# wathiede/pbrt

Measured on AMD Instinct MI355X. Metric: Msamples/sec (rays/sec) at 1/2/4/8 GPUs; PSNR vs CPU reference, higher is better.
Workload: dtype f32

## Files before the change

### include/pbrt_hip_debug.h

```cpp
#ifndef PBRT_HIP_DEBUG_H
#define PBRT_HIP_DEBUG_H
#include "pbrt_hip.h"
#ifdef __cplusplus
extern "C" {
#endif

int pbrt_hip_scene_canonical_info(const pbrt_hip_scene *scene, uint32_t *ready, double *build_ms);
int pbrt_hip_scene_optimize_cost(const pbrt_hip_scene *scene, double *before, double *after, uint32_t *undone);
int pbrt_hip_scene_export_quads(const pbrt_hip_scene *scene, uint32_t *quads, uint32_t cap_nodes, uint32_t *n_quads,
                                uint32_t *order);
int pbrt_hip_scene_export_bvh(const pbrt_hip_scene *scene, uint32_t *nodes , uint32_t *order);
int pbrt_hip_scene_walk_info(const pbrt_hip_scene *scene, uint32_t *quad_nodes, uint32_t *stack_need);
int pbrt_hip_render_stack_plan(uint32_t stack_need, uint32_t *lds_rows, uint32_t *waves_per_cu, uint32_t *overflow_entries);
int pbrt_hip_rccl_library(char *path, size_t cap);
int pbrt_hip_bvh_build_host(const float *P, uint32_t n_verts, const uint32_t *idx, uint32_t n_tris,
                            uint32_t *nodes , uint32_t *order, uint32_t *n_nodes,
                            uint32_t *depth);

int pbrt_hip_quad_build_host(const float *P, uint32_t n_verts, const uint32_t *idx, uint32_t n_tris, int split_leaves,
                             uint32_t *quads, uint32_t cap_nodes, uint32_t *n_quads, uint32_t *stack_need);
#define PBRT_HIP_TREE_SAH 0u
#define PBRT_HIP_TREE_REINSERT 2u
#define PBRT_HIP_TREE_DEFAULT 0xffffffffu
int pbrt_hip_quad_build_host_ex(const float *P, uint32_t n_verts, const uint32_t *idx, uint32_t n_tris, int split_leaves,
                                uint32_t tree, uint32_t *quads, uint32_t cap_nodes, uint32_t *n_quads, uint32_t *stack_need,
                                uint32_t *order, float *root_box, uint32_t *n_refs, float *exact_boxes);

void pbrt_hip_sobol_matrices(uint32_t *out_4096_words);
int pbrt_hip_envmap_tables(const float *rgb, uint32_t width, uint32_t height, float *marginal, float *conditional, float *p_uv);
int pbrt_hip_envmap_eval_host(const float *rgb, uint32_t width, uint32_t height, const float world_to_light[9], int64_t n, const float *u12,
                              float *d, uint32_t *texel, float *le, float *pdf);
int pbrt_hip_envmap_eval_device(pbrt_hip_scene *scene, int64_t n, const float *u12, float *d, uint32_t *texel, float *le, float *pdf);

#define PBRT_HIP_BLOCK_SIN 0u
#define PBRT_HIP_BLOCK_COS 1u
#define PBRT_HIP_BLOCK_ATAN_POS 2u
// ... 25 lines not shown
```

### pbrt_amd/_lib.py

```python
import ctypes as C
import os

from .build import LIB_PATH


class Material(C.Structure):
    _fields_ = [("type", C.c_uint32), ("k", C.c_float * 3), ("le", C.c_float * 3), ("kd_tex", C.c_uint32)]


class Texture(C.Structure):
    _fields_ = [("type", C.c_uint32), ("tex1", C.c_float * 3), ("tex2", C.c_float * 3), ("su", C.c_float), ("sv", C.c_float),
                ("du", C.c_float), ("dv", C.c_float), ("pad", C.c_uint32 * 5)]


class EnvMap(C.Structure):
    _fields_ = [("type", C.c_uint32), ("width", C.c_uint32), ("height", C.c_uint32), ("reserved", C.c_uint32), ("rgb", C.POINTER(C.c_float)),
                ("world_to_light", C.c_float * 9), ("pad", C.c_uint32)]


class Normals(C.Structure):
    _fields_ = [("type", C.c_uint32), ("n_tris", C.c_uint32), ("reserved", C.c_uint32 * 2), ("tri_n", C.POINTER(C.c_float)),
                ("pad", C.c_uint32 * 10)]


# ... 31 lines not shown
        ("nodes_visited", C.c_uint64), ("tris_tested", C.c_uint64), ("kernel_ms", C.c_double),
        ("samples", C.c_uint64),
    ]


_f, _u32, _i32, _i64, _u64, _vp = C.c_float, C.c_uint32, C.c_int32, C.c_int64, C.c_uint64, C.c_void_p
_pf, _pu32, _pi32, _pi64, _pu64, _pu8 = (C.POINTER(t) for t in (_f, _u32, _i32, _i64, _u64, C.c_uint8))
SYMBOLS = {
    "pbrt_hip_device_count": (C.c_int, []),
    "pbrt_hip_last_error": (C.c_char_p, []),
    "pbrt_hip_version": (C.c_char_p, []),
    "pbrt_hip_build_id": (C.c_char_p, []),
    "pbrt_hip_scene_create": (C.c_int, [C.POINTER(SceneDesc), C.c_int, C.POINTER(_vp)]),
    "pbrt_hip_scene_create_ex": (C.c_int, [C.POINTER(SceneDesc), C.c_int, _u32, C.POINTER(_vp)]),
    "pbrt_hip_scene_build_info": (C.c_int, [_vp, _pu32, C.POINTER(C.c_double)]),
    "pbrt_hip_scene_canonical_info": (C.c_int, [_vp, _pu32, C.POINTER(C.c_double)]),
    "pbrt_hip_scene_optimize_info": (C.c_int, [_vp, _pu32, _pu32, C.POINTER(C.c_double)]),
    "pbrt_hip_rccl_library": (C.c_int, [C.c_char_p, C.c_size_t]),
    "pbrt_hip_scene_optimize_cost": (C.c_int, [_vp, C.POINTER(C.c_double), C.POINTER(C.c_double), _pu32]),
    "pbrt_hip_scene_export_quads": (C.c_int, [_vp, _pu32, _u32, _pu32, _pu32]),
    "pbrt_hip_scene_destroy": (None, [_vp]),
    "pbrt_hip_scene_info": (C.c_int, [_vp, _pu32, _pu32, _pu32, _pu64]),
    "pbrt_hip_render_stack_plan": (C.c_int, [C.c_uint32, _pu32, _pu32, _pu32]),
    "pbrt_hip_scene_export_bvh": (C.c_int, [_vp, _pu32, _pu32]),
    "pbrt_hip_scene_walk_info": (C.c_int, [_vp, _pu32, _pu32]),
    "pbrt_hip_bvh_build_host": (C.c_int, [_pf, _u32, _pu32, _u32, _pu32, _pu32, _pu32, _pu32]),
    "pbrt_hip_quad_build_host": (C.c_int, [_pf, _u32, _pu32, _u32, C.c_int, _pu32, _u32, _pu32, _pu32]),
    "pbrt_hip_quad_build_host_ex": (C.c_int, [_pf, _u32, _pu32, _u32, C.c_int, _u32, _pu32, _u32, _pu32, _pu32, _pu32, _pf, _pu32, _pf]),
    "pbrt_hip_render": (C.c_int, [_vp, C.POINTER(RenderDesc), _pf, C.POINTER(Stats)]),
    "pbrt_hip_render_device": (C.c_int, [_vp, C.POINTER(RenderDesc), _vp, _vp]),
    "pbrt_hip_render_prepare": (C.c_int, [_vp, C.POINTER(RenderDesc)]),
    "pbrt_hip_render_wait": (C.c_int, [_vp, C.POINTER(Stats)]),
    "pbrt_hip_film_assemble_device": (C.c_int, [_vp, _vp, _u32, _u32, _vp, _vp]),
    "pbrt_hip_render_buffer_bytes": (_i64, [_vp, C.POINTER(RenderDesc)]),
    "pbrt_hip_render_acc": (C.c_int, [_vp, C.POINTER(RenderDesc), _pi64, C.POINTER(Stats)]),
    "pbrt_hip_film_from_acc_device": (C.c_int, [_vp, _vp, _vp, _vp]),
    "pbrt_hip_film_from_acc": (None, [_pi64, _i64, _pf]),
    "pbrt_hip_sobol_matrices": (None, [_pu32]),
    "pbrt_hip_slab_floats": (_i64, [_i32, _i32, _pf, _u32, _u32]),
    "pbrt_hip_slab_pixel_index": (C.c_int, [_i32, _i32, _pf, _u32, _u32, _pi64]),
    "pbrt_hip_multi_create": (C.c_int, [C.POINTER(SceneDesc), C.c_int, _u32, C.POINTER(_vp)]),
    "pbrt_hip_multi_gpus": (C.c_int, [_vp]),
    "pbrt_hip_multi_render": (C.c_int, [_vp, C.POINTER(RenderDesc), _pf, C.POINTER(Stats)]),
    "pbrt_hip_multi_film_device": (C.c_int, [_vp, C.POINTER(_vp)]),
    "pbrt_hip_multi_destroy": (None, [_vp]),
    "pbrt_hip_render_multi": (C.c_int, [C.POINTER(SceneDesc), C.POINTER(RenderDesc), C.c_int, _pf, C.POINTER(Stats)]),
# ... 71 lines not shown
```

### pbrt_amd/csrc/capi_render.cpp

```cpp
#include <hip/hip_runtime.h>

#include <cmath>
#include <cstdio>
#include <cstdlib>
#include <cstring>
#include <algorithm>
#include <limits>
#include <string>
#include <vector>

#include "../../include/pbrt_hip.h"
#include "capi_internal.hpp"
#include "device_types.h"
#include "host_math.hpp"
#include "rgb_xyz.hpp"

using namespace pbrt_hip;

namespace pbrt_hip {
namespace {
inline float filter_radius(float w) { return w == 0.f ? 0.5f : w; }
inline bool filter_is_wide(float rx, float ry) { return rx != 0.5f || ry != 0.5f; }
void sample_bounds(const int32_t c[4], float rx, float ry, int32_t sb[4]) {
  sb[0] = (int32_t)std::floor(((float)c[0] + 0.5f) - rx);
// ... 46 lines not shown
  int32_t b[4];
  film_cropped_bounds(xres, yres, crop, b);
  return make_shard_bounds(b, rank, world);
}
struct TileRect {
  int32_t x0, y0, w, h;
};
TileRect super_tile(const Shard &sh, uint32_t rank, uint32_t world, uint32_t j) {
  const uint32_t t = rank + j * world;
  const int32_t x0 = (int32_t)(t % sh.stx) * 64, y0 = (int32_t)(t / sh.stx) * 64;
  return {x0, y0, sh.w - x0 < 64 ? sh.w - x0 : 64, sh.h - y0 < 64 ? sh.h - y0 : 64};
}

uint32_t tuning(const char *name, uint32_t dflt, long cap = 64) {
  const char *v = debug_knob(name);
  if (!v || !*v) return dflt;
  long x = std::strtol(v, nullptr, 10);
  return x < 0 ? 0u : (x > cap ? (uint32_t)cap : (uint32_t)x);
}
constexpr uint32_t kMinWalkers = 36, kMinWalkersShallow = 20, kShallowStackNeed = 16, kMinParked = 16;
constexpr uint32_t kRenderWavesPerCuSpheres = 12;
constexpr uint32_t kRenderWavesPerCuEnv = 16;
constexpr uint32_t kRenderWavesPerCuN = 16;
RenderStackPlan stack_plan(uint32_t quad_stack_need) {
  static const bool force_overflow = debug_knob("PBRT_HIP_FORCE_OVERFLOW_VARIANT") != nullptr;
  static const bool prefer_lds = debug_knob("PBRT_HIP_PREFER_LDS_STACK") != nullptr;
  return render_stack_plan(quad_stack_need, force_overflow, prefer_lds);
}
bool is_table_sampler(uint32_t sampler) { return sampler == PBRT_HIP_SAMPLER_SOBOL_ND || sampler == PBRT_HIP_SAMPLER_HALTON; }

int check_render_desc(const pbrt_hip_scene *s, const pbrt_hip_render_desc *r) {
  if (!s || !r) return fail(PBRT_HIP_ERR_INVALID, "render: null argument");
  if (r->spp_x == 0 || r->spp_y == 0) return fail(PBRT_HIP_ERR_INVALID, "render: spp_x and spp_y must be >= 1");
  if (r->world_size == 0 || r->rank >= r->world_size) return fail(PBRT_HIP_ERR_INVALID, "render: rank must be < world_size");
  if (r->integrator > PBRT_HIP_INTEGRATOR_PATH_MIS) return fail(PBRT_HIP_ERR_INVALID, "render: unknown integrator");
  if (r->sampler > PBRT_HIP_SAMPLER_HALTON) return fail(PBRT_HIP_ERR_INVALID, "render: unknown sampler");
  const bool counting = (r->flags & (PBRT_HIP_FLAG_COUNTERS | PBRT_HIP_FLAG_WALK_COUNTERS)) != 0u;
  if (is_table_sampler(r->sampler) && counting)
    return fail(PBRT_HIP_ERR_INVALID, "render: the counter flags are not available with the Sobol' / Halton samplers (samplers 2, 3)");
  if ((uint64_t)r->spp_x * (uint64_t)r->spp_y > PBRT_HIP_MAX_SPP)
    return fail(PBRT_HIP_ERR_LIMIT, "render: more than 2^20 samples per pixel");
  if (r->max_depth > PBRT_HIP_MAX_DEPTH) return fail(PBRT_HIP_ERR_LIMIT, "render: maxdepth above 1023");
  const float fx = filter_radius(r->filter_xwidth), fy = filter_radius(r->filter_ywidth);
  if (!(fx > 0.f) || !(fy > 0.f) || !std::isfinite(fx) || !std::isfinite(fy)) return fail(PBRT_HIP_ERR_INVALID, "render: the filter radii must be positive");
  if (fx > 16.f || fy > 16.f) return fail(PBRT_HIP_ERR_LIMIT, "render: filter radius above 16 pixels");
  const bool wide = filter_is_wide(fx, fy);
  if (wide && counting)
    return fail(PBRT_HIP_ERR_INVALID, "render: the counter flags need the default box filter (radius 0.5)");
  if (s->normals && counting)
    return fail(PBRT_HIP_ERR_LIMIT, "render: the counter flags are not available for a scene with shading normals");
// ... 16 lines not shown
  return PBRT_HIP_OK;
}

uint32_t partials_passes(uint32_t n_local, uint32_t n_chunks) {
  if (n_local == 0) return 1;
  const uint64_t cap_bytes = (uint64_t)std::max<uint32_t>(1u, tuning("PBRT_HIP_PARTIALS_CAP_KB", 2u << 20, 1l << 30)) << 10;
  const uint64_t per_tile = 4096ull * n_chunks * 16ull;
  uint64_t tiles = std::max<uint64_t>(1, cap_bytes / per_tile);
  tiles = std::min<uint64_t>(tiles, ((1ull << 32) - 1) / (4096ull * n_chunks));
  return (uint32_t)((n_local + tiles - 1) / tiles);
}
int render_launch(pbrt_hip_scene *s, const pbrt_hip_render_desc *r, const FilmGeom &fg, const Shard &sh, RenderLaunch *out) {
  RenderLaunch L{};
  L.spheres = s->dev.n_spheres > 0;
  L.counters = (r->flags & PBRT_HIP_FLAG_COUNTERS) ? kCountExact : ((r->flags & PBRT_HIP_FLAG_WALK_COUNTERS) ? kCountWalk : kCountNone);
  L.wide = fg.wide;
  L.table_sampler = is_table_sampler(r->sampler);
  L.mis = r->integrator == PBRT_HIP_INTEGRATOR_PATH_MIS;
  L.textured = s->textured;
  L.glass = s->glass;
  L.env = s->env;
  L.normals = s->normals;
  const bool shallow = s->dev.quad_stack_need <= kShallowStackNeed;
  L.plan = stack_plan(s->dev.quad_stack_need);
  L.lds_bytes = L.plan.rows * 256u;
  const bool default_path = L.counters == kCountNone && !L.wide && !L.table_sampler && !L.mis && !L.textured && !L.glass && !L.env && !L.normals;
  L.steps = default_path && !L.plan.overflow && shallow ? 2u : PBRT_STEPS_PER_CHECK;
  if (L.counters == kCountExact) {
    const int ce = ensure_canonical(s);
    if (ce) return ce;
    const uint32_t held = s->bvh.depth > 0 ? s->bvh.depth - 1 : 0;
    L.exact_rows = held > 40 ? 64 : held > 32 ? 40 : held > 26 ? 32 : held > 20 ? 26 : 20;
    L.lds_bytes = L.exact_rows * 512u;
  }
  L.waves_per_cu = (L.spheres || L.glass) ? std::min(kRenderWavesPerCuSpheres, L.plan.waves_per_cu) : L.plan.waves_per_cu;
  if (L.env) L.waves_per_cu = std::min(kRenderWavesPerCuEnv, L.plan.waves_per_cu);
  if (L.normals) L.waves_per_cu = std::min(kRenderWavesPerCuN, L.plan.waves_per_cu);
  L.chunk_shift = sample_chunk_shift(r->spp_x * r->spp_y);
  const uint32_t n_chunks = 1u << L.chunk_shift;
  L.passes = fg.wide ? 1u : partials_passes(sh.n_local, n_chunks);
  L.pass_tiles = (sh.n_local + L.passes - 1) / L.passes;
  if ((uint64_t)L.pass_tiles * 4096u * n_chunks >= (1ull << 32)) return fail(PBRT_HIP_ERR_LIMIT, "render: film too large for 32-bit item numbers");
  if ((uint64_t)r->world_size * L.passes >= (1ull << 32)) return fail(PBRT_HIP_ERR_LIMIT, "render: world_size x passes does not fit 32 bits");
  L.n_workgroups = std::min<uint32_t>(L.pass_tiles * 64u * n_chunks, std::max<uint32_t>(1u, tuning("PBRT_HIP_RENDER_WORKGROUPS", s->n_cu * L.waves_per_cu, 1 << 20)));
  L.min_walkers = tuning("PBRT_HIP_MIN_WALKERS", shallow ? kMinWalkersShallow : kMinWalkers);
  L.min_parked = tuning("PBRT_HIP_MIN_PARKED", kMinParked);
  *out = L;
  return PBRT_HIP_OK;
}
// ... 18 lines not shown
    if (s->d_partials.n / 4 > need) s->d_partials.release();
    HIP_TRY(s->d_partials.grow(need));
  }
  HIP_TRY(s->d_stack_overflow.grow((size_t)L.n_workgroups * 64 * L.plan.extra_entries));
  return PBRT_HIP_OK;
}
void scene_render_params(const pbrt_hip_scene *s, RenderParams *R) {
  R->tri_uv = s->d_tri_uv.p;
  R->textures = s->d_textures.p;
  R->glass = s->d_glass.p;
  R->env_texels = s->d_env_texels.p;
  R->env_marginal = s->d_env_marginal.p;
  R->env_conditional = s->d_env_conditional.p;
  R->env_w = s->env_w; R->env_h = s->env_h;
  for (int k = 0; k < 9; k++) R->env_m[k] = s->env_m[k];
  for (int k = 0; k < 3; k++) R->env_c[k] = s->env_c[k];
  R->tri_n = s->d_tri_n.p;
}
}

extern "C" {

int pbrt_hip_render_stack_plan(uint32_t stack_need, uint32_t *lds_rows, uint32_t *waves_per_cu, uint32_t *overflow_entries) {
  const RenderStackPlan p = stack_plan(stack_need);
  if (lds_rows) *lds_rows = p.rows;
  if (waves_per_cu) *waves_per_cu = p.waves_per_cu;
  if (overflow_entries) *overflow_entries = p.extra_entries;
  return PBRT_HIP_OK;
}

int pbrt_hip_envmap_eval_device(pbrt_hip_scene *s, int64_t n, const float *u12, float *d, uint32_t *texel, float *le, float *pdf) {
  if (!s) return fail(PBRT_HIP_ERR_INVALID, "envmap_eval_device: null scene");
  if (!s->env) return fail(PBRT_HIP_ERR_INVALID, "envmap_eval_device: the scene has no environment map");
  if (n < 0 || (n && !d)) return fail(PBRT_HIP_ERR_INVALID, "envmap_eval_device: null argument");
  if (n == 0) return PBRT_HIP_OK;
  return guarded([&]() -> int {
    HIP_TRY(hipSetDevice(s->device));
    DevBuf<float> d_u, d_d, d_le, d_pdf;
    DevBuf<uint32_t> d_texel;
    HIP_TRY(d_d.alloc(3 * (size_t)n));
    HIP_TRY(d_le.alloc(3 * (size_t)n));
    HIP_TRY(d_pdf.alloc((size_t)n));
    HIP_TRY(d_texel.alloc((size_t)n));
    if (u12) {
      HIP_TRY(d_u.alloc(2 * (size_t)n));
      HIP_TRY(hipMemcpyAsync(d_u.p, u12, 8 * (size_t)n, hipMemcpyHostToDevice, s->stream));
    } else {
      HIP_TRY(hipMemcpyAsync(d_d.p, d, 12 * (size_t)n, hipMemcpyHostToDevice, s->stream));
// ... 386 lines not shown
```

### pbrt_amd/csrc/device_types.h

```cpp
#pragma once
#include <stdint.h>

#include <hip/hip_runtime.h>

#include <cstdlib>

namespace pbrt_hip {

inline const char *debug_knob(const char *name) {
  const char *on = std::getenv("PBRT_HIP_DEBUG_KNOBS");
  if (!on || !*on || (on[0] == '0' && !on[1])) return nullptr;
  return std::getenv(name);
}

#ifdef PBRT_QUAD_LDS_STACK
constexpr uint32_t kQuadLdsStack = PBRT_QUAD_LDS_STACK, kQuadLdsStackOvf = PBRT_QUAD_LDS_STACK;
#else
constexpr uint32_t kQuadLdsStack = 40, kQuadLdsStackOvf = 30;
#endif
constexpr uint32_t kLdsGranule = 1280u;
constexpr uint32_t kLdsBytesPerCu = 160u * 1024u;
#ifndef PBRT_TRI_STRIDE
#define PBRT_TRI_STRIDE 4
#endif
constexpr uint32_t kTriStride = PBRT_TRI_STRIDE;
#ifndef PBRT_STEPS_PER_CHECK
#define PBRT_STEPS_PER_CHECK 3
#endif
#ifndef PBRT_RENDER_MAX_WAVES_PER_CU
#define PBRT_RENDER_MAX_WAVES_PER_CU 20
#endif
constexpr uint32_t kRenderMaxWavesPerCu = PBRT_RENDER_MAX_WAVES_PER_CU;

constexpr uint32_t kEmptyLeafRef = 0x80000000u;
constexpr uint32_t kLeafRef = 0x80000000u;

constexpr uint32_t kMaxSampleChunks = 16u, kMinSamplesPerChunk = 32u;
inline uint32_t sample_chunk_shift(uint32_t spp) {
  uint32_t kb = 0;
  while ((2u << kb) <= kMaxSampleChunks && (2u << kb) * kMinSamplesPerChunk <= spp) kb++;
  return kb;
}

constexpr uint32_t kSobolNdRequests = 64u;

struct RenderStackPlan {
  uint32_t rows;
  bool overflow;
  uint32_t waves_per_cu;
  uint32_t extra_entries;
};
inline RenderStackPlan render_stack_plan(uint32_t quad_stack_need, bool force_overflow, bool prefer_lds = false) {
  RenderStackPlan p;
  const uint32_t need_rows = quad_stack_need + 2u;
  auto waves = [](uint32_t rows) {
    const uint32_t bytes = (rows * 256u + kLdsGranule - 1u) / kLdsGranule * kLdsGranule, w = kLdsBytesPerCu / bytes;
    return w > kRenderMaxWavesPerCu ? kRenderMaxWavesPerCu : w;
  };
  p.rows = need_rows < 8u ? 8u : need_rows;
  p.overflow = force_overflow || need_rows > kQuadLdsStack || (waves(p.rows) < waves(kQuadLdsStackOvf) && !prefer_lds);
  if (p.overflow) p.rows = kQuadLdsStackOvf;
  p.waves_per_cu = waves(p.rows);
  p.extra_entries = p.overflow && need_rows > p.rows ? need_rows - p.rows : 0u;
  return p;
}
constexpr uint32_t kIntersectLdsStack = 20;
constexpr uint32_t kIntersectWavesPerWorkgroup = 4, kIntersectMaxWorkgroups = 256 * 16;
inline uint32_t intersect_workgroups(int64_t n_rays) {
  const int64_t w = (n_rays + 255) / 256;
  return w > kIntersectMaxWorkgroups ? kIntersectMaxWorkgroups : (uint32_t)w;
}
inline uint32_t intersect_overflow_entries(uint32_t quad_stack_need) {
  return quad_stack_need + 2u > kIntersectLdsStack ? quad_stack_need + 2u - kIntersectLdsStack : 0u;
}

struct DevScene {
  const uint4 *nodes;
  const uint4 *quads;
  uint32_t quad_stack_need;
  const float4 *tris;
  const float4 *mats;
  const float4 *lights;
  const float4 *spheres;
  uint32_t n_nodes, n_tris, n_spheres, n_lights;
  float n_lights_f;
// ... 124 lines not shown
```

### pbrt_amd/csrc/kernel_path.hpp

```cpp
#pragma once
#include "envmap_core.hpp"
#include "kernel_walk.hpp"

namespace pbrt_hip {
namespace {

__device__ __forceinline__ bool sample_light(const DevScene &S, uint32_t li, V3 po, V3 nf, V3 kd, float u1, float u2,
                                             float nLf, V3 &Ld, V3 &wi, float &tmax, const bool mis = false) {
  const float4 l0 = S.lights[5 * li];
  const float4 l3 = S.lights[5 * li + 3];
  const uint32_t type = __float_as_uint(l0.x);
  const V3 p0 = {l0.y, l0.z, l0.w};
  const V3 lc = xyz(l3);
  const V3 f = kd * kInvPi;
  if (type == 0u) {
    V3 dv = p0 - po;
    float dist2 = dot(dv, dv);
    if (!(dist2 > 0.f)) return false;
    float dist = sqrtf(dist2);
    wi = dv / dist;
    float cs = dot(wi, nf);
    if (!(cs > 0.f)) return false;
    float scale = (cs / dist2) * nLf;
    Ld = (f * lc) * scale;
// ... 75 lines not shown
    scale = scale * mis_weight_light(pl, pbl);
  }
  Ld = (f * (mk(R.env_c[0], R.env_c[1], R.env_c[2]) * xyz(tx))) * scale;
  tmax = kInf;
  return true;
}

enum : uint32_t { ST_NEW = 0, ST_CLOSEST = 1, ST_SHADOW = 2, ST_DONE = 3, ST_FETCH = 4 };

#ifndef PBRT_RENDER_WAVES_PER_SIMD
#define PBRT_RENDER_WAVES_PER_SIMD 5
#endif

struct PathState {
  V3 L, beta;
  V3 wi_next;
  Pcg rng;
  uint32_t s, bounces;
  bool specular, cont;
};
struct LaneRecords {
  char *base;
  uint32_t off;
};
constexpr int32_t kRecL = -2048, kRecBeta = -1024, kRecWi = 0, kRecLpend = 1024, kRecSum = 2048;
__device__ __forceinline__ float4 rec_load(const LaneRecords &r, int32_t k) {
  uint32_t o = r.off;
  asm volatile("" : "+v"(o));
  return *reinterpret_cast<const float4 *>(r.base + o + k);
}
__device__ __forceinline__ void rec_store(const LaneRecords &r, int32_t k, float4 v) {
  uint32_t o = r.off;
  asm volatile("" : "+v"(o));
  *reinterpret_cast<float4 *>(r.base + o + k) = v;
}
__device__ __forceinline__ void path_store(const LaneRecords &rec, const PathState &P) {
  rec_store(rec, kRecL, make_float4(P.L.x, P.L.y, P.L.z,
                                    __uint_as_float(P.s | (P.bounces << 20) | (P.specular ? 1u << 30 : 0u) | (P.cont ? 1u << 31 : 0u))));
  rec_store(rec, kRecBeta, make_float4(P.beta.x, P.beta.y, P.beta.z, __uint_as_float((uint32_t)P.rng.state)));
  rec_store(rec, kRecWi, make_float4(P.wi_next.x, P.wi_next.y, P.wi_next.z, __uint_as_float((uint32_t)(P.rng.state >> 32))));
}
__device__ __forceinline__ void path_load(const LaneRecords &rec, PathState &P) {
  const float4 a = rec_load(rec, kRecL), b = rec_load(rec, kRecBeta), c = rec_load(rec, kRecWi);
  P.L = {a.x, a.y, a.z};
  P.beta = {b.x, b.y, b.z};
  P.wi_next = {c.x, c.y, c.z};
  const uint32_t w = __float_as_uint(a.w);
  P.s = w & 0xfffffu;
  P.bounces = (w >> 20) & 0x3ffu;
  P.specular = (w >> 30) & 1u;
  P.cont = (w >> 31) & 1u;
  P.rng.state = (uint64_t)__float_as_uint(b.w) | ((uint64_t)__float_as_uint(c.w) << 32);
}

__device__ __forceinline__ uint32_t chunk_begin(uint32_t c, uint32_t spp, uint32_t kb) { return (c * spp) >> kb; }
__device__ __forceinline__ uint32_t mix32(uint32_t v) {
  v ^= v >> 16; v *= 0x7feb352du; v ^= v >> 15; v *= 0x846ca68bu; v ^= v >> 16;
  return v;
}
__device__ __forceinline__ float halton_dim(const uint32_t *tab, uint32_t d, uint32_t i, uint32_t key, uint32_t spp_mask) {
  const uint4 t = reinterpret_cast<const uint4 *>(tab)[d];
  const uint32_t b = t.x;
  uint32_t h = mix32(key + (d + 1u) * 0x9e3779b9u);
  if (b == 2u) return fminf(kOneMinusEps, (float)(__builtin_bitreverse32(i) ^ h) * 2.3283064365386963e-10f);
  uint32_t v = 0u, n = i, pw = 1u;
  do {
// ... 90 lines not shown
```

### pbrt_amd/csrc/kernels.hip

```cpp
#include "kernel_path.hpp"
#include "rgb_xyz.hpp"
#include "with_bools.hpp"

namespace pbrt_hip {
namespace {

template <bool SPH, bool COUNT, bool EXACT, int STACK, int STEPS = PBRT_STEPS_PER_CHECK, bool WIDE = false, bool SND = false>
__global__ void __launch_bounds__(64, (COUNT ? 1 : (SPH ? 3 : PBRT_RENDER_WAVES_PER_SIMD))) render_kernel(const DevScene S, const RenderParams R) {
  constexpr bool MIS = false, TEX = false, GLS = false;
  constexpr bool ENV = false;
  constexpr bool NRM = false;
  (void)MIS;
  (void)GLS;
  (void)ENV;
#include "render_body.inc"
}

#ifndef PBRT_INTERSECT_WAVES_PER_SIMD
#define PBRT_INTERSECT_WAVES_PER_SIMD 8
#endif
template <bool SPH, bool COUNT, int STACK>
__global__ void __launch_bounds__(256, (COUNT ? 1 : (SPH ? 4 : PBRT_INTERSECT_WAVES_PER_SIMD))) intersect_kernel(const DevScene S, const RayBatch B, const int any_hit) {
  __shared__ uint32_t lds_stack[4][COUNT ? STACK : kIntersectLdsStack][64];
  __shared__ float lds_tn[COUNT ? 4 : 1][COUNT ? STACK : 1][64];
  const uint32_t lane = threadIdx.x & 63u, wave = threadIdx.x >> 6;
  uint32_t *stk = &lds_stack[wave][0][lane];
  float *stkt = &lds_tn[COUNT ? wave : 0][0][lane];
  uint32_t *ovf = B.stack_overflow + ((size_t)blockIdx.x * 4u + (uint32_t)__builtin_amdgcn_readfirstlane(wave)) * B.stack_overflow_entries * 64u;
  const TravTuning tune = {B.min_walkers, B.min_parked};
  unsigned long long cn = 0, ct = 0;
  EXP_PROBE_INIT_BLOCK();
  const int64_t stride = (int64_t)gridDim.x * 256;
  int64_t next = (int64_t)blockIdx.x * 256 + threadIdx.x, idx = 0;
  bool have = false;
// ... 155 lines not shown
  };
  if (L.counters == kCountExact)
    return with_bools([&](auto SPH) {
      switch (L.exact_rows) {
        case 20: return go(render_kernel<SPH, true, true, 20>);
        case 26: return go(render_kernel<SPH, true, true, 26>);
        case 32: return go(render_kernel<SPH, true, true, 32>);
        case 40: return go(render_kernel<SPH, true, true, 40>);
        case 64: return go(render_kernel<SPH, true, true, 64>);
      }
      return hipErrorInvalidValue;
    }, L.spheres);
  if (L.glass || L.mis || L.textured || (L.table_sampler && L.wide)) return launch_render_x(S, R, L, st);
  const bool experiment = kExperimentLaunch && L.counters == kCountNone && !L.wide && !L.table_sampler;
  hipError_t e = hipSuccess;
  if (experiment && experiment_launch_begin(&e)) return e;
  e = with_bools([&](auto SPH, auto OVF, auto COUNT, auto SND, auto WIDE) {
    constexpr int STACK = OVF ? (int)kQuadLdsStackOvf : 0;
    if constexpr ((COUNT && (SND || WIDE)) || (SND && WIDE)) {
      return hipErrorInvalidValue;
    } else if constexpr (!COUNT && !SND && !WIDE && STACK == 0) {
      return go(L.steps == 2 ? render_kernel<SPH, false, false, 0, 2> : render_kernel<SPH, false, false, 0>);
    } else {
      return go(render_kernel<SPH, COUNT, false, STACK, PBRT_STEPS_PER_CHECK, WIDE, SND>);
    }
  }, L.spheres, L.plan.overflow, L.counters == kCountWalk, L.table_sampler, L.wide);
  if (experiment) experiment_launch_end(st);
  return e;
}

hipError_t launch_intersect(const DevScene &S, const RayBatch &B, bool any_hit, uint32_t bvh_depth, hipStream_t st) {
  if (B.n == 0) return hipSuccess;
  const dim3 grid(intersect_workgroups(B.n)), block(64 * kIntersectWavesPerWorkgroup);
  const hipError_t e = with_bools([&](auto SPH, auto COUNT) {
    hipLaunchKernelGGL((bvh_depth <= 32 ? intersect_kernel<SPH, COUNT, 32> : intersect_kernel<SPH, COUNT, 64>), grid, block, 0, st, S, B, any_hit ? 1 : 0);
    return hipGetLastError();
  }, S.n_spheres > 0, B.counters != nullptr);
  if (kExperimentLaunch) experiment_launch_end(st);
  return e;
}

hipError_t launch_pack_tris(const float *P, const uint32_t *idx, const uint16_t *mat_id, const uint32_t *order,
                            uint32_t n_prims, uint32_t n_tris, const float4 *spheres, float4 *tris, hipStream_t stream) {
  if (n_prims == 0) return hipSuccess;
  hipLaunchKernelGGL(pack_tris_kernel, dim3((n_prims + 255) / 256), dim3(256), 0, stream, P, idx, mat_id, order, n_prims, n_tris, spheres,
                     tris);
// ... 29 lines not shown
```

### pbrt_amd/csrc/kernels_env.hip

```cpp
#include "kernel_path.hpp"
#include "with_bools.hpp"

namespace pbrt_hip {
namespace {

#ifndef PBRT_ENV_WAVES_PER_SIMD
#define PBRT_ENV_WAVES_PER_SIMD 4
#endif
template <bool SPH, int STACK, bool MIS, bool TEX, bool SND>
__global__ void __launch_bounds__(64, PBRT_ENV_WAVES_PER_SIMD) render_kernel_env(const DevScene S, const RenderParams R) {
  constexpr bool COUNT = false, EXACT = false, WIDE = false, GLS = true, ENV = true;
  constexpr bool NRM = false;
  constexpr int STEPS = PBRT_STEPS_PER_CHECK;
#include "render_body.inc"
}

__global__ void envmap_eval_kernel(const RenderParams R, int64_t n, const float *u12, float *d, uint32_t *texel, float *le, float *pdf) {
  const int64_t i = (int64_t)blockIdx.x * blockDim.x + threadIdx.x;
  if (i >= n) return;
  const envmap::Map m = env_map(R);
  float st;
  uint32_t t;
  if (u12) {
    float x, y, z;
    t = envmap::sample(m, u12[2 * i], u12[2 * i + 1], &x, &y, &z, &st);
    d[3 * i] = x; d[3 * i + 1] = y; d[3 * i + 2] = z;
  } else {
    t = envmap::lookup(m, d[3 * i], d[3 * i + 1], d[3 * i + 2], &st);
  }
  const float4 tx = m.texels[t];
  if (texel) texel[i] = t;
  if (le) { le[3 * i] = tx.x; le[3 * i + 1] = tx.y; le[3 * i + 2] = tx.z; }
  if (pdf) pdf[i] = envmap::pdf_omega(tx.w, st);
}

// ... 20 lines not shown
```

### pbrt_amd/csrc/kernels_n.hip

```cpp
#include "kernel_path.hpp"
#include "with_bools.hpp"

namespace pbrt_hip {
namespace {

#ifndef PBRT_NRM_WAVES_PER_SIMD
#define PBRT_NRM_WAVES_PER_SIMD 4
#endif
template <bool SPH, int STACK, bool MIS, bool TEX, bool SND, bool ENV>
__global__ void __launch_bounds__(64, PBRT_NRM_WAVES_PER_SIMD) render_kernel_n(const DevScene S, const RenderParams R) {
  constexpr bool COUNT = false, EXACT = false, WIDE = false, GLS = true, NRM = true;
  constexpr int STEPS = PBRT_STEPS_PER_CHECK;
#include "render_body.inc"
}

__global__ void pack_nrm_kernel(const float *tri_n, const uint32_t *order, uint32_t n_prims, uint32_t n_tris, float4 *out) {
  const uint32_t slot = blockIdx.x * blockDim.x + threadIdx.x;
  if (slot >= n_prims) return;
  const uint32_t t = order[slot];
  for (int v = 0; v < 3; v++) {
    const float *q = tri_n + 9 * (size_t)t + 3 * v;
    out[3u * slot + v] = t < n_tris ? make_float4(q[0], q[1], q[2], 0.f) : make_float4(0.f, 0.f, 0.f, 0.f);
  }
}

__global__ void __launch_bounds__(256) shading_normal_eval_kernel(int64_t n, const float *in, float *out) {
  const int64_t i = (int64_t)blockIdx.x * blockDim.x + threadIdx.x;
  if (i >= n) return;
  const float *x = in + 17 * i;
  const V3 sn_n0 = mk(x[0], x[1], x[2]), sn_n1 = mk(x[3], x[4], x[5]), sn_n2 = mk(x[6], x[7], x[8]);
  const V3 ng = mk(x[9], x[10], x[11]);
  const float sn_b1 = x[12], sn_b2 = x[13];
  const V3 wo = mk(x[14], x[15], x[16]);
#include "shading_normal.inc"
// ... 30 lines not shown
```

### pbrt_amd/csrc/kernels_x.hip

```cpp
#include "kernel_path.hpp"
#include "with_bools.hpp"

namespace pbrt_hip {
namespace {

template <bool SPH, int STACK, bool MIS, bool TEX, bool SND, bool WIDE, bool GLS = false>
__global__ void __launch_bounds__(64, ((SPH || GLS) ? 3 : PBRT_RENDER_WAVES_PER_SIMD)) render_kernel_x(const DevScene S, const RenderParams R) {
  constexpr bool COUNT = false, EXACT = false;
  constexpr bool ENV = false;
  constexpr bool NRM = false;
  constexpr int STEPS = PBRT_STEPS_PER_CHECK;
  (void)ENV;
#include "render_body.inc"
}

}

hipError_t launch_render_x(const DevScene &S, const RenderParams &R, const RenderLaunch &L, hipStream_t st) {
  if (R.n_items == 0) return hipSuccess;
  if (L.counters != kCountNone) return hipErrorInvalidValue;
  return with_bools([&](auto SPH, auto OVF, auto MIS, auto TEX, auto SND, auto WIDE, auto GLS) {
    constexpr int STACK = OVF ? (int)kQuadLdsStackOvf : 0;
    if constexpr (GLS || MIS || TEX || (SND && WIDE)) {
      hipLaunchKernelGGL((render_kernel_x<SPH, STACK, MIS, TEX, SND, WIDE, GLS>), dim3(L.n_workgroups), dim3(64), L.lds_bytes, st, S, R);
      return hipGetLastError();
    } else {
      return hipErrorInvalidValue;
    }
  }, L.spheres, L.plan.overflow, L.mis, L.textured, L.table_sampler, L.wide, L.glass);
}

}
```

### pbrt_amd/csrc/render_body.inc

```
  extern __shared__ uint32_t lds_stack[];
  const uint32_t lane = threadIdx.x;
  uint32_t *stk = lds_stack + lane;
  float *stkt = reinterpret_cast<float *>(lds_stack + (EXACT ? STACK : 0) * 64) + lane;
  uint32_t *ovf = R.stack_overflow + (size_t)blockIdx.x * R.stack_overflow_entries * 64u;

  const int32_t W = R.sw, H = R.sh;
  const uint32_t stx = (uint32_t)(W + 63) >> 6;
  const uint64_t seq0 = R.seed * (uint64_t)R.seq_w * (uint64_t)R.seq_h;
  uint32_t item = 0;
  auto pixel_xy = [&](uint32_t q, int32_t &xr, int32_t &yr) {
    const uint32_t tsup = R.rank + (q >> 12) * R.world;
    const uint32_t ty = stx == 1u ? tsup : __umulhi(tsup, R.stx_recip), tx = tsup - ty * stx;
    xr = (int32_t)(tx * 64u + ((q >> 6) & 7u) * 8u + (q & 7u));
    yr = (int32_t)(ty * 64u + ((q >> 9) & 7u) * 8u + ((q >> 3) & 7u));
  };
  const uint32_t kb = R.chunk_shift, chunk_mask = (1u << kb) - 1u;
  auto item_pixel = [&](uint32_t it) { return ((it >> (6u + kb)) << 6) | (it & 63u); };
  auto slab_pos = [](uint32_t q) {
    return (size_t)(q >> 12) * 4096u + (((q >> 9) & 7u) * 8u + ((q >> 3) & 7u)) * 64u + ((q >> 6) & 7u) * 8u + (q & 7u);
  };
  const bool sobol = SND ? true : R.sampler == 1u;
  const bool halton = SND && R.sampler == 3u;
  const uint32_t spp = R.spp_x * R.spp_y;
  const uint32_t spp_mask = R.spp_mask;
  const uint32_t nL = S.n_lights;
  const float nLf = S.n_lights_f;
  const bool direct_only = R.integrator == 1u;
  const TravTuning tune = {R.min_walkers, R.min_parked};

  const LaneRecords rec = {reinterpret_cast<char *>(R.lane_state + (size_t)blockIdx.x * 320u + 128u), lane * 16u};
  uint32_t state = ST_FETCH;
  if (WIDE) wide_slots_clear(R.wide_slots, lane);
  uint32_t region = blockIdx.x % R.n_regions;
  unsigned long long c_cam = 0, c_bounce = 0, c_shadow = 0, c_nodes = 0, c_tris = 0;
  Trav T;
  T.o = mk(0.f, 0.f, 0.f);
  T.d = mk(0.f, 0.f, 1.f);
  T.tmax = 0.f;
  T.cur = kDone;
  T.sp = 0;
  T.any = 0;
  T.h = HitRec{kInf, kNoPrim, kNoPrim, 0.f, 0.f};

  EXP_PROBE_INIT(lane);
  for (;;) {
    EXP_PROBE_LANES(4, state != ST_DONE && T.cur == kDone);
    const bool serve = state != ST_DONE && T.cur == kDone;
    PathState P;
    bool launch = false, launch_any = false;
    V3 ro = T.o, rd = T.d;
    float rtmax = kInf;
    int32_t xr = 0, yr = 0;
    if (serve && state != ST_FETCH) {
      path_load(rec, P);
      pixel_xy(item_pixel(item), xr, yr);
      P.rng.inc = ((((seq0 + (uint64_t)(R.seq_y0 + yr) * (uint64_t)R.seq_w + (uint64_t)(R.seq_x0 + xr)) << kb) + ((item >> 6) & chunk_mask)) << 1) | 1u;
      PROBE_SEC(1);
      if (state != ST_NEW) {
        bool advance = false;
        if (state == ST_SHADOW) {
          EXP_DEBUG_PIXEL("HIP s %u   shadow Lpend %08x occluded %u tmax %a\n", P.s, __float_as_uint(rec_load(rec, kRecLpend).x), T.any >> 1, T.tmax);
          if (T.any != 3u) {
            const float4 lp = rec_load(rec, kRecLpend);
            P.L = P.L + mk(lp.x, lp.y, lp.z);
          }
          advance = true;
        } else {
          const HitRec h = T.h;
          const bool hit = h.prim != kNoPrim;
          EXP_DEBUG_PIXEL("HIP s %u bounce %u prim %u t %08x b1 %a b2 %a L %08x beta %08x\n", P.s, P.bounces, h.prim, __float_as_uint(h.t), h.b1, h.b2,
                          __float_as_uint(P.L.x), __float_as_uint(P.beta.x));
          EXP_DEBUG_PIXEL("HIP s %u   ray o %a %a %a d %a %a %a\n", P.s, T.o.x, T.o.y, T.o.z, T.d.x, T.d.y, T.d.z);
          V3 p = {0.f, 0.f, 0.f}, ng = {0.f, 0.f, 1.f};
          float4 m0 = {0.f, 0.f, 0.f, 0.f}, m1 = {0.f, 0.f, 0.f, 0.f};
          float tri_area = 0.f;
          float4 gl = {0.f, 0.f, 0.f, 1.f};
          const V3 wo = -T.d;
// ... 318 lines not shown
            const uint32_t sx = P.s - sy * R.spp_x;
            jx = fminf(((float)sx + u1) * R.inv_nx, kOneMinusEps);
            jy = fminf(((float)sy + u2) * R.inv_ny, kOneMinusEps);
          }
          const float fx = (float)(R.sx0 + xr) + jx, fy = (float)(R.sy0 + yr) + jy;
          if (WIDE) rec_store(rec, kRecSum, make_float4(fx, fy, 0.f, 0.f));
          const V3 dc = unit(mk(fx * S.cam_ax + S.cam_bx, fy * S.cam_ay + S.cam_by, 1.0f));
          rd = {(S.c2w[0] * dc.x + S.c2w[1] * dc.y) + S.c2w[2] * dc.z,
                (S.c2w[4] * dc.x + S.c2w[5] * dc.y) + S.c2w[6] * dc.z,
                (S.c2w[8] * dc.x + S.c2w[9] * dc.y) + S.c2w[10] * dc.z};
          ro = {S.c2w[3], S.c2w[7], S.c2w[11]};
          rtmax = kInf;
          P.L = {0.f, 0.f, 0.f};
          P.beta = {1.f, 1.f, 1.f};
          P.specular = false;
          P.bounces = 0;
          state = ST_CLOSEST;
          launch = true;
          launch_any = false;
          if (COUNT) c_cam++;
        }
      }
      PROBE_SEC(7);
      path_store(rec, P);
      EXP_RAY_LOG(launch, ro, rd, rtmax, launch_any);
      if (launch) trav_begin<EXACT>(S, T, stk, ro, rd, rtmax, launch_any, c_nodes);
    }
    PROBE_SEC(8);
    if (__ballot(state != ST_DONE) == 0ull) break;
    wave_prio(PBRT_PRIO_ARITH);
    trav_run<EXACT, COUNT, ((!EXACT && STACK != 0) ? (uint32_t)STACK : 0u), STEPS, SPH>(S, T, stk, stkt, ovf, state != ST_DONE, tune, c_nodes, c_tris);
    wave_prio(PBRT_PRIO_SERVICE);
    PROBE_SEC(0);
  }

  EXP_PROBE_FINI(lane);
  if (COUNT) {
    unsigned long long v[5] = {c_cam, c_bounce, c_shadow, c_nodes, c_tris};
    for (int i = 0; i < 5; i++) {
      unsigned long long x = v[i];
      for (int off = 32; off > 0; off >>= 1) x += __shfl_down(x, off, 64);
      if (lane == 0) atomicAdd(&R.counters[i], x);
    }
  }
```

Measured before the change: 454.8.

## Keep per-lane path records in LDS behind the traversal stack for overflow kernels

In the overflow-stack render kernel on the default path, the three per-lane path-state records (L, beta, wi) now live in LDS, placed after a shortened traversal stack, instead of in global lane_state memory. The goal is to replace global-memory loads and stores at each path service step with LDS accesses. In exchange, the LDS walk stack shrinks by 12 rows, so more stack entries spill to the global overflow area. The LDS budget per wave and the waves-per-CU calculation now include the record rows, and a host check verifies that the plan matches the kernel variant.

```diff
diff --git a/include/pbrt_hip_debug.h b/include/pbrt_hip_debug.h
--- a/include/pbrt_hip_debug.h
+++ b/include/pbrt_hip_debug.h
@@ -12,6 +12,8 @@
 int pbrt_hip_scene_export_bvh(const pbrt_hip_scene *scene, uint32_t *nodes , uint32_t *order);
 int pbrt_hip_scene_walk_info(const pbrt_hip_scene *scene, uint32_t *quad_nodes, uint32_t *stack_need);
 int pbrt_hip_render_stack_plan(uint32_t stack_need, uint32_t *lds_rows, uint32_t *waves_per_cu, uint32_t *overflow_entries);
+int pbrt_hip_render_stack_layout(uint32_t stack_need, uint32_t *stack_rows, uint32_t *record_bytes, uint32_t *waves_per_cu,
+                                 uint32_t *overflow_entries);
 int pbrt_hip_rccl_library(char *path, size_t cap);
 int pbrt_hip_bvh_build_host(const float *P, uint32_t n_verts, const uint32_t *idx, uint32_t n_tris,
                             uint32_t *nodes , uint32_t *order, uint32_t *n_nodes,
diff --git a/pbrt_amd/_lib.py b/pbrt_amd/_lib.py
--- a/pbrt_amd/_lib.py
+++ b/pbrt_amd/_lib.py
@@ -77,6 +77,7 @@
     "pbrt_hip_scene_destroy": (None, [_vp]),
     "pbrt_hip_scene_info": (C.c_int, [_vp, _pu32, _pu32, _pu32, _pu64]),
     "pbrt_hip_render_stack_plan": (C.c_int, [C.c_uint32, _pu32, _pu32, _pu32]),
+    "pbrt_hip_render_stack_layout": (C.c_int, [C.c_uint32, _pu32, _pu32, _pu32, _pu32]),
     "pbrt_hip_scene_export_bvh": (C.c_int, [_vp, _pu32, _pu32]),
     "pbrt_hip_scene_walk_info": (C.c_int, [_vp, _pu32, _pu32]),
     "pbrt_hip_bvh_build_host": (C.c_int, [_pf, _u32, _pu32, _u32, _pu32, _pu32, _pu32, _pu32]),
diff --git a/pbrt_amd/csrc/capi_render.cpp b/pbrt_amd/csrc/capi_render.cpp
--- a/pbrt_amd/csrc/capi_render.cpp
+++ b/pbrt_amd/csrc/capi_render.cpp
@@ -92,10 +92,10 @@
 constexpr uint32_t kRenderWavesPerCuSpheres = 12;
 constexpr uint32_t kRenderWavesPerCuEnv = 16;
 constexpr uint32_t kRenderWavesPerCuN = 16;
-RenderStackPlan stack_plan(uint32_t quad_stack_need) {
+RenderStackPlan stack_plan(uint32_t quad_stack_need, bool lds_records) {
   static const bool force_overflow = debug_knob("PBRT_HIP_FORCE_OVERFLOW_VARIANT") != nullptr;
   static const bool prefer_lds = debug_knob("PBRT_HIP_PREFER_LDS_STACK") != nullptr;
-  return render_stack_plan(quad_stack_need, force_overflow, prefer_lds);
+  return render_stack_plan(quad_stack_need, force_overflow, prefer_lds, lds_records);
 }
 bool is_table_sampler(uint32_t sampler) { return sampler == PBRT_HIP_SAMPLER_SOBOL_ND || sampler == PBRT_HIP_SAMPLER_HALTON; }
 
@@ -158,9 +158,9 @@
   L.env = s->env;
   L.normals = s->normals;
   const bool shallow = s->dev.quad_stack_need <= kShallowStackNeed;
-  L.plan = stack_plan(s->dev.quad_stack_need);
-  L.lds_bytes = L.plan.rows * 256u;
   const bool default_path = L.counters == kCountNone && !L.wide && !L.table_sampler && !L.mis && !L.textured && !L.glass && !L.env && !L.normals;
+  L.plan = stack_plan(s->dev.quad_stack_need, default_path);
+  L.lds_bytes = (L.plan.rows + L.plan.record_rows) * 256u;
   L.steps = default_path && !L.plan.overflow && shallow ? 2u : PBRT_STEPS_PER_CHECK;
   if (L.counters == kCountExact) {
     const int ce = ensure_canonical(s);
@@ -225,8 +225,17 @@
 extern "C" {
 
 int pbrt_hip_render_stack_plan(uint32_t stack_need, uint32_t *lds_rows, uint32_t *waves_per_cu, uint32_t *overflow_entries) {
-  const RenderStackPlan p = stack_plan(stack_need);
+  const RenderStackPlan p = stack_plan(stack_need, false);
   if (lds_rows) *lds_rows = p.rows;
+  if (waves_per_cu) *waves_per_cu = p.waves_per_cu;
+  if (overflow_entries) *overflow_entries = p.extra_entries;
+  return PBRT_HIP_OK;
+}
+
+int pbrt_hip_render_stack_layout(uint32_t stack_need, uint32_t *stack_rows, uint32_t *record_bytes, uint32_t *waves_per_cu, uint32_t *overflow_entries) {
+  const RenderStackPlan p = stack_plan(stack_need, true);
+  if (stack_rows) *stack_rows = p.rows;
+  if (record_bytes) *record_bytes = p.record_rows * 256u;
   if (waves_per_cu) *waves_per_cu = p.waves_per_cu;
   if (overflow_entries) *overflow_entries = p.extra_entries;
   return PBRT_HIP_OK;
diff --git a/pbrt_amd/csrc/device_types.h b/pbrt_amd/csrc/device_types.h
--- a/pbrt_amd/csrc/device_types.h
+++ b/pbrt_amd/csrc/device_types.h
@@ -18,6 +18,15 @@
 #else
 constexpr uint32_t kQuadLdsStack = 40, kQuadLdsStackOvf = 30;
 #endif
+constexpr uint32_t kPathRecordRows = 12u;
+#ifdef PBRT_PATH_RECORDS_HBM
+constexpr bool kLdsPathRecords = false;
+#else
+constexpr bool kLdsPathRecords = true;
+#endif
+constexpr uint32_t kQuadLdsWalkRows = kQuadLdsStackOvf >= kPathRecordRows + 8u ? kQuadLdsStackOvf - kPathRecordRows : kQuadLdsStackOvf;
+static_assert(kQuadLdsWalkRows >= 8u, "PBRT_QUAD_LDS_STACK: the walk's LDS part needs at least 8 rows");
+static_assert((kQuadLdsWalkRows * 256u) % 16u == 0u && (kPathRecordRows * 256u) == 3u * 1024u, "path records 0..2: three 16-byte-aligned 1 KB rows behind the stack");
 constexpr uint32_t kLdsGranule = 1280u;
 constexpr uint32_t kLdsBytesPerCu = 160u * 1024u;
 #ifndef PBRT_TRI_STRIDE
@@ -49,8 +58,9 @@
   bool overflow;
   uint32_t waves_per_cu;
   uint32_t extra_entries;
-};
-inline RenderStackPlan render_stack_plan(uint32_t quad_stack_need, bool force_overflow, bool prefer_lds = false) {
+  uint32_t record_rows;
+};
+inline RenderStackPlan render_stack_plan(uint32_t quad_stack_need, bool force_overflow, bool prefer_lds = false, bool lds_records = false) {
   RenderStackPlan p;
   const uint32_t need_rows = quad_stack_need + 2u;
   auto waves = [](uint32_t rows) {
@@ -59,8 +69,9 @@
   };
   p.rows = need_rows < 8u ? 8u : need_rows;
   p.overflow = force_overflow || need_rows > kQuadLdsStack || (waves(p.rows) < waves(kQuadLdsStackOvf) && !prefer_lds);
-  if (p.overflow) p.rows = kQuadLdsStackOvf;
-  p.waves_per_cu = waves(p.rows);
+  p.record_rows = p.overflow && lds_records && kLdsPathRecords ? kPathRecordRows : 0u;
+  if (p.overflow) p.rows = p.record_rows ? kQuadLdsWalkRows : kQuadLdsStackOvf;
+  p.waves_per_cu = waves(p.rows + p.record_rows);
   p.extra_entries = p.overflow && need_rows > p.rows ? need_rows - p.rows : 0u;
   return p;
 }
diff --git a/pbrt_amd/csrc/kernel_path.hpp b/pbrt_amd/csrc/kernel_path.hpp
--- a/pbrt_amd/csrc/kernel_path.hpp
+++ b/pbrt_amd/csrc/kernel_path.hpp
@@ -121,6 +121,7 @@
 struct LaneRecords {
   char *base;
   uint32_t off;
+  uint32_t lds;
 };
 constexpr int32_t kRecL = -2048, kRecBeta = -1024, kRecWi = 0, kRecLpend = 1024, kRecSum = 2048;
 __device__ __forceinline__ float4 rec_load(const LaneRecords &r, int32_t k) {
@@ -133,14 +134,34 @@
   asm volatile("" : "+v"(o));
   *reinterpret_cast<float4 *>(r.base + o + k) = v;
 }
+struct alignas(16) LdsRec { float x, y, z, w; };
+typedef __attribute__((address_space(3))) LdsRec lds_rec;
+template <bool LDS>
+__device__ __forceinline__ float4 path_rec_load(const LaneRecords &r, int32_t k) {
+  if (!LDS) return rec_load(r, k);
+  uint32_t o = r.off;
+  asm volatile("" : "+v"(o));
+  const lds_rec *p = (const lds_rec *)(uintptr_t)(r.lds + (uint32_t)(k - kRecL) + o);
+  return make_float4(p->x, p->y, p->z, p->w);
+}
+template <bool LDS>
+__device__ __forceinline__ void path_rec_store(const LaneRecords &r, int32_t k, float4 v) {
+  if (!LDS) { rec_store(r, k, v); return; }
+  uint32_t o = r.off;
+  asm volatile("" : "+v"(o));
+  lds_rec *p = (lds_rec *)(uintptr_t)(r.lds + (uint32_t)(k - kRecL) + o);
+  p->x = v.x; p->y = v.y; p->z = v.z; p->w = v.w;
+}
+template <bool LDS = false>
 __device__ __forceinline__ void path_store(const LaneRecords &rec, const PathState &P) {
-  rec_store(rec, kRecL, make_float4(P.L.x, P.L.y, P.L.z,
+  path_rec_store<LDS>(rec, kRecL, make_float4(P.L.x, P.L.y, P.L.z,
                                     __uint_as_float(P.s | (P.bounces << 20) | (P.specular ? 1u << 30 : 0u) | (P.cont ? 1u << 31 : 0u))));
-  rec_store(rec, kRecBeta, make_float4(P.beta.x, P.beta.y, P.beta.z, __uint_as_float((uint32_t)P.rng.state)));
-  rec_store(rec, kRecWi, make_float4(P.wi_next.x, P.wi_next.y, P.wi_next.z, __uint_as_float((uint32_t)(P.rng.state >> 32))));
-}
+  path_rec_store<LDS>(rec, kRecBeta, make_float4(P.beta.x, P.beta.y, P.beta.z, __uint_as_float((uint32_t)P.rng.state)));
+  path_rec_store<LDS>(rec, kRecWi, make_float4(P.wi_next.x, P.wi_next.y, P.wi_next.z, __uint_as_float((uint32_t)(P.rng.state >> 32))));
+}
+template <bool LDS = false>
 __device__ __forceinline__ void path_load(const LaneRecords &rec, PathState &P) {
-  const float4 a = rec_load(rec, kRecL), b = rec_load(rec, kRecBeta), c = rec_load(rec, kRecWi);
+  const float4 a = path_rec_load<LDS>(rec, kRecL), b = path_rec_load<LDS>(rec, kRecBeta), c = path_rec_load<LDS>(rec, kRecWi);
   P.L = {a.x, a.y, a.z};
   P.beta = {b.x, b.y, b.z};
   P.wi_next = {c.x, c.y, c.z};
diff --git a/pbrt_amd/csrc/kernels.hip b/pbrt_amd/csrc/kernels.hip
--- a/pbrt_amd/csrc/kernels.hip
+++ b/pbrt_amd/csrc/kernels.hip
@@ -5,11 +5,15 @@
 namespace pbrt_hip {
 namespace {
 
+constexpr bool render_kernel_lds_records(bool count, bool exact, int stack, bool wide, bool snd) {
+  return kLdsPathRecords && !count && !exact && !wide && !snd && stack != 0;
+}
 template <bool SPH, bool COUNT, bool EXACT, int STACK, int STEPS = PBRT_STEPS_PER_CHECK, bool WIDE = false, bool SND = false>
 __global__ void __launch_bounds__(64, (COUNT ? 1 : (SPH ? 3 : PBRT_RENDER_WAVES_PER_SIMD))) render_kernel(const DevScene S, const RenderParams R) {
   constexpr bool MIS = false, TEX = false, GLS = false;
   constexpr bool ENV = false;
   constexpr bool NRM = false;
+  constexpr bool LREC = render_kernel_lds_records(COUNT, EXACT, STACK, WIDE, SND);
   (void)MIS;
   (void)GLS;
   (void)ENV;
@@ -211,6 +215,7 @@
     } else if constexpr (!COUNT && !SND && !WIDE && STACK == 0) {
       return go(L.steps == 2 ? render_kernel<SPH, false, false, 0, 2> : render_kernel<SPH, false, false, 0>);
     } else {
+      if (render_kernel_lds_records(COUNT, false, STACK, WIDE, SND) != (L.plan.record_rows != 0u)) return hipErrorInvalidValue;
       return go(render_kernel<SPH, COUNT, false, STACK, PBRT_STEPS_PER_CHECK, WIDE, SND>);
     }
   }, L.spheres, L.plan.overflow, L.counters == kCountWalk, L.table_sampler, L.wide);
diff --git a/pbrt_amd/csrc/kernels_env.hip b/pbrt_amd/csrc/kernels_env.hip
--- a/pbrt_amd/csrc/kernels_env.hip
+++ b/pbrt_amd/csrc/kernels_env.hip
@@ -11,6 +11,7 @@
 __global__ void __launch_bounds__(64, PBRT_ENV_WAVES_PER_SIMD) render_kernel_env(const DevScene S, const RenderParams R) {
   constexpr bool COUNT = false, EXACT = false, WIDE = false, GLS = true, ENV = true;
   constexpr bool NRM = false;
+  constexpr bool LREC = false;
   constexpr int STEPS = PBRT_STEPS_PER_CHECK;
 #include "render_body.inc"
 }
diff --git a/pbrt_amd/csrc/kernels_n.hip b/pbrt_amd/csrc/kernels_n.hip
--- a/pbrt_amd/csrc/kernels_n.hip
+++ b/pbrt_amd/csrc/kernels_n.hip
@@ -10,6 +10,7 @@
 template <bool SPH, int STACK, bool MIS, bool TEX, bool SND, bool ENV>
 __global__ void __launch_bounds__(64, PBRT_NRM_WAVES_PER_SIMD) render_kernel_n(const DevScene S, const RenderParams R) {
   constexpr bool COUNT = false, EXACT = false, WIDE = false, GLS = true, NRM = true;
+  constexpr bool LREC = false;
   constexpr int STEPS = PBRT_STEPS_PER_CHECK;
 #include "render_body.inc"
 }
diff --git a/pbrt_amd/csrc/kernels_x.hip b/pbrt_amd/csrc/kernels_x.hip
--- a/pbrt_amd/csrc/kernels_x.hip
+++ b/pbrt_amd/csrc/kernels_x.hip
@@ -9,6 +9,7 @@
   constexpr bool COUNT = false, EXACT = false;
   constexpr bool ENV = false;
   constexpr bool NRM = false;
+  constexpr bool LREC = false;
   constexpr int STEPS = PBRT_STEPS_PER_CHECK;
   (void)ENV;
 #include "render_body.inc"
diff --git a/pbrt_amd/csrc/render_body.inc b/pbrt_amd/csrc/render_body.inc
--- a/pbrt_amd/csrc/render_body.inc
+++ b/pbrt_amd/csrc/render_body.inc
@@ -28,7 +28,9 @@
   const bool direct_only = R.integrator == 1u;
   const TravTuning tune = {R.min_walkers, R.min_parked};
 
-  const LaneRecords rec = {reinterpret_cast<char *>(R.lane_state + (size_t)blockIdx.x * 320u + 128u), lane * 16u};
+  constexpr uint32_t WROWS = (!EXACT && STACK != 0) ? (LREC ? kQuadLdsWalkRows : (uint32_t)STACK) : 0u;
+  const LaneRecords rec = {reinterpret_cast<char *>(R.lane_state + (size_t)blockIdx.x * 320u + 128u), lane * 16u,
+                           LREC ? lds_addr(lds_stack) + WROWS * kRowBytes : 0u};
   uint32_t state = ST_FETCH;
   if (WIDE) wide_slots_clear(R.wide_slots, lane);
   uint32_t region = blockIdx.x % R.n_regions;
@@ -52,7 +54,7 @@
     float rtmax = kInf;
     int32_t xr = 0, yr = 0;
     if (serve && state != ST_FETCH) {
-      path_load(rec, P);
+      path_load<LREC>(rec, P);
       pixel_xy(item_pixel(item), xr, yr);
       P.rng.inc = ((((seq0 + (uint64_t)(R.seq_y0 + yr) * (uint64_t)R.seq_w + (uint64_t)(R.seq_x0 + xr)) << kb) + ((item >> 6) & chunk_mask)) << 1) | 1u;
       PROBE_SEC(1);
@@ -417,14 +419,14 @@
         }
       }
       PROBE_SEC(7);
-      path_store(rec, P);
+      path_store<LREC>(rec, P);
       EXP_RAY_LOG(launch, ro, rd, rtmax, launch_any);
       if (launch) trav_begin<EXACT>(S, T, stk, ro, rd, rtmax, launch_any, c_nodes);
     }
     PROBE_SEC(8);
     if (__ballot(state != ST_DONE) == 0ull) break;
     wave_prio(PBRT_PRIO_ARITH);
-    trav_run<EXACT, COUNT, ((!EXACT && STACK != 0) ? (uint32_t)STACK : 0u), STEPS, SPH>(S, T, stk, stkt, ovf, state != ST_DONE, tune, c_nodes, c_tris);
+    trav_run<EXACT, COUNT, WROWS, STEPS, SPH>(S, T, stk, stkt, ovf, state != ST_DONE, tune, c_nodes, c_tris);
     wave_prio(PBRT_PRIO_SERVICE);
     PROBE_SEC(0);
   }
```

Result: faster. 467.8 (median of 6 runs) (+2.8%).
